# ziyaad30/ForwardTacotron

Measured on AMD Instinct MI355X. Metric: mel_frames_per_sec_train_step, higher is better.
Workload: dtype f32

## Files before the change

### forwardtacotron_amd/csrc/ft_lr.hip

```cpp
#include "ft_common.h"

namespace {

__global__ __launch_bounds__(64) void ft_lr_scan_kernel(float* dur, int Tx, int* cum, int* total) {
  const int b = blockIdx.x, lane = threadIdx.x;
  float* d = dur + (long)b * Tx;
  int* c = cum + (long)b * (Tx + 1);
  int carry = 0;
  for (int j0 = 0; j0 < Tx; j0 += 64) {
    int j = j0 + lane;
    int r = 0;
    if (j < Tx) {
      float v = d[j];
      if (v < 0.f) {
        v = 0.f;
        d[j] = 0.f;
      }
      r = (int)(long)(v + 0.5f);
    }
    int s = r;
#pragma unroll
    for (int o = 1; o < 64; o <<= 1) {
      int u = __shfl_up(s, o, 64);
      if (lane >= o) s += u;
    }
    if (j < Tx) c[j] = carry + s - r;
    carry += __shfl(s, 63, 64);
  }
  if (lane == 0) {
    c[Tx] = carry;
    total[b] = carry;
  }
}

__global__ __launch_bounds__(64) void ft_gen_durations_kernel(float* dur, const long* __restrict__ x_len, int Tx,
                                                              long* __restrict__ mel_len, int* bad) {
  const int b = blockIdx.x, lane = threadIdx.x;
  float* d = dur + (long)b * Tx;
  long Lb = x_len[b];
  if (Lb < 1 || Lb > Tx) {
    if (lane == 0) atomicOr(bad, 1);
    Lb = Lb < 1 ? 1 : Tx;
  }
  const int L = (int)Lb;
  long tr = 0;
  for (int j = lane; j < L; j += 64) tr += (long)d[j];
#pragma unroll
  for (int o = 32; o > 0; o >>= 1) tr += __shfl_xor(tr, o, 64);
  const bool fallback = tr <= 0;
  long total = 0;
  for (int j = lane; j < Tx; j += 64) {
    float v = 0.f;
    if (j < L) {
      v = fallback ? 2.f : d[j];
      if (v < 0.f) v = 0.f;
    }
    d[j] = v;
    total += (long)(v + 0.5f);
  }
#pragma unroll
  for (int o = 32; o > 0; o >>= 1) total += __shfl_xor(total, o, 64);
  if (lane == 0) mel_len[b] = total;
}

template <int FR>
__global__ __launch_bounds__(256) void ft_lr_expand_kernel(const float* __restrict__ x, const int* __restrict__ cum,
                                                           float* __restrict__ y, int* __restrict__ src_idx,
                                                           int Tx, int Tm, int C, int vec, long y_bs, long y_ts,
                                                           const float* __restrict__ pad_row) {
  __shared__ int src[FR];
  const int b = blockIdx.y;
  const int t0 = blockIdx.x * FR;
  const int* c = cum + (long)b * (Tx + 1);
  if (threadIdx.x < FR) {
    int t = t0 + threadIdx.x;
    int tok = -1;
    if (t < Tm && t < c[Tx]) {
      int lo = 0, hi = Tx - 1;
      while (lo < hi) {
        int mid = (lo + hi + 1) >> 1;
        if (c[mid] <= t) lo = mid; else hi = mid - 1;
      }
      tok = lo;
    }
    src[threadIdx.x] = tok;
    if (t < Tm && src_idx) src_idx[(long)b * Tm + t] = tok;
  }
  __syncthreads();
  const int wave = threadIdx.x >> 6, lane = threadIdx.x & 63;
  for (int f = wave; f < FR; f += 4) {
    int t = t0 + f;
    if (t >= Tm) break;
    int tok = src[f];
    float* yr = y + ((long)b * y_bs + (long)t * y_ts) * C;
    if (vec) {
      const float4* xr = reinterpret_cast<const float4*>(tok < 0 ? pad_row : x + ((long)b * Tx + tok) * C);
      float4* y4 = reinterpret_cast<float4*>(yr);
      for (int i = lane; i < C / 4; i += 64) y4[i] = xr ? xr[i] : make_float4(0.f, 0.f, 0.f, 0.f);
    } else {
      const float* xr = tok < 0 ? pad_row : x + ((long)b * Tx + tok) * C;
      for (int i = lane; i < C; i += 64) yr[i] = xr ? xr[i] : 0.f;
    }
  }
}

__global__ __launch_bounds__(256) void ft_lr_bwd_cols_kernel(const float* __restrict__ dy, const int* __restrict__ cum,
                                                             float* __restrict__ dx, float* __restrict__ dtail, int B,
                                                             int Tx, int Tm, int C, long dy_bs, long dy_ts) {
  const int wave = threadIdx.x >> 6, lane = threadIdx.x & 63;
  const long row = (long)blockIdx.x * 4 + wave;
  const int col = (blockIdx.y * 64 + lane) * 4;
  const long ntok = (long)B * Tx;
  if (row >= ntok + (dtail ? B : 0) || col >= C) return;
  const bool tail = row >= ntok;
  const int b = tail ? (int)(row - ntok) : (int)(row / Tx), j = tail ? Tx : (int)(row - (long)b * Tx);
  const int* c = cum + (long)b * (Tx + 1);
  int f0 = c[j], f1 = tail ? Tm : c[j + 1];
  if (f1 > Tm) f1 = Tm;
  float4 a = make_float4(0.f, 0.f, 0.f, 0.f);
  const float* src = dy + ((long)b * dy_bs + (long)f0 * dy_ts) * C + col;
  const long step = dy_ts * C;
  for (int t = f0; t < f1; t += 4, src += 4 * step) {
    const float4 z = make_float4(0.f, 0.f, 0.f, 0.f);
    const float4 g0 = *reinterpret_cast<const float4*>(src);
    const float4 g1 = t + 1 < f1 ? *reinterpret_cast<const float4*>(src + step) : z;
    const float4 g2 = t + 2 < f1 ? *reinterpret_cast<const float4*>(src + 2 * step) : z;
    const float4 g3 = t + 3 < f1 ? *reinterpret_cast<const float4*>(src + 3 * step) : z;
    a.x = (((a.x + g0.x) + g1.x) + g2.x) + g3.x;
    a.y = (((a.y + g0.y) + g1.y) + g2.y) + g3.y;
    a.z = (((a.z + g0.z) + g1.z) + g2.z) + g3.z;
    a.w = (((a.w + g0.w) + g1.w) + g2.w) + g3.w;
  }
  *reinterpret_cast<float4*>((tail ? dtail + (long)b * C : dx + row * C) + col) = a;
}

__global__ __launch_bounds__(256) void ft_lr_bwd_kernel(const float* __restrict__ dy, const int* __restrict__ cum,
                                                        float* __restrict__ dx, int B, int Tx, int Tm, int C, int vec) {
  const int wave = threadIdx.x >> 6, lane = threadIdx.x & 63;
  long row = (long)blockIdx.x * 4 + wave;
  if (row >= (long)B * Tx) return;
  int b = (int)(row / Tx), j = (int)(row - (long)b * Tx);
  const int* c = cum + (long)b * (Tx + 1);
  int f0 = c[j], f1 = c[j + 1];
  if (f1 > Tm) f1 = Tm;
  float* dxr = dx + row * C;
  if (vec) {
    for (int i = lane; i < C / 4; i += 64) {
      float4 a = make_float4(0.f, 0.f, 0.f, 0.f);
      for (int t = f0; t < f1; ++t) {
        float4 g = reinterpret_cast<const float4*>(dy + ((long)b * Tm + t) * C)[i];
        a.x += g.x; a.y += g.y; a.z += g.z; a.w += g.w;
      }
      reinterpret_cast<float4*>(dxr)[i] = a;
    }
  } else {
    for (int i = lane; i < C; i += 64) {
      float a = 0.f;
      for (int t = f0; t < f1; ++t) a += dy[((long)b * Tm + t) * C + i];
      dxr[i] = a;
    }
  }
}

}

int ft_gen_durations_impl(float* dur, const long* x_len, int B, int Tx, long* mel_len, int* bad, hipStream_t stream) {
  if (B <= 0) return FT_OK;
  hipLaunchKernelGGL(ft_gen_durations_kernel, dim3(B), dim3(64), 0, stream, dur, x_len, Tx, mel_len, bad);
  return ft_check_launch("gen_durations");
}

int ft_lr_scan_impl(float* dur, int B, int Tx, int* cum, int* total, hipStream_t stream) {
  FT_REQUIRE(B >= 0 && Tx >= 0, "lr_scan: bad dims");
  if (B == 0) return FT_OK;
  hipLaunchKernelGGL(ft_lr_scan_kernel, dim3(B), dim3(64), 0, stream, dur, Tx, cum, total);
  return ft_check_launch("lr_scan");
}

int ft_lr_expand_impl(const float* x, const int* cum, float* y, int* src_idx, int B, int Tx, int Tm, int C,
                      hipStream_t stream, int y_time_major, const float* pad_row) {
  FT_REQUIRE(B >= 0 && Tx >= 0 && Tm >= 0 && C >= 0, "lr_expand: bad dims");
  if (B == 0 || Tm == 0 || C == 0) return FT_OK;
  FT_REQUIRE(Tx > 0, "lr_expand: Tm > 0 requires Tx > 0");
  int vec = (C % 4 == 0) && ((uintptr_t)x % 16 == 0) && ((uintptr_t)y % 16 == 0) && ((uintptr_t)pad_row % 16 == 0);
  constexpr int FR = 16;
  hipLaunchKernelGGL(ft_lr_expand_kernel<FR>, dim3(ft_cdiv(Tm, FR), B), dim3(256), 0, stream, x, cum, y, src_idx,
                     Tx, Tm, C, vec, y_time_major ? 1L : (long)Tm, y_time_major ? (long)B : 1L, pad_row);
  return ft_check_launch("lr_expand");
}

int ft_lr_bwd_impl(const float* dy, const int* cum, float* dx, int B, int Tx, int Tm, int C, hipStream_t stream,
                   int dy_time_major, float* dtail) {
  FT_REQUIRE(B >= 0 && Tx >= 0 && Tm >= 0 && C >= 0, "lr_bwd: bad dims");
  if (B == 0 || Tx == 0 || C == 0) return FT_OK;
  int vec = (C % 4 == 0) && ((uintptr_t)dy % 16 == 0) && ((uintptr_t)dx % 16 == 0);
  if (dy_time_major || dtail || (vec && C >= 1024)) {
    FT_REQUIRE(vec && (uintptr_t)dtail % 16 == 0, "lr_bwd: this form needs C %% 4 == 0 and 16-byte aligned buffers");
    hipLaunchKernelGGL(ft_lr_bwd_cols_kernel, dim3(ft_cdiv((long)B * Tx + (dtail ? B : 0), 4), ft_cdiv(C, 256)), dim3(256),
                       0, stream, dy, cum, dx, dtail, B, Tx, Tm, C, dy_time_major ? 1L : (long)Tm,
                       dy_time_major ? (long)B : 1L);
    return ft_check_launch("lr_bwd");
  }
  hipLaunchKernelGGL(ft_lr_bwd_kernel, dim3(ft_cdiv((long)B * Tx, 4)), dim3(256), 0, stream, dy, cum, dx, B, Tx, Tm,
                     C, vec);
  return ft_check_launch("lr_bwd");
}
```

### forwardtacotron_amd/csrc/ft_rnn.hip

```cpp
#include <stdlib.h>

#include <string.h>

#include "ft_gemm.h"
#include "ft_rnn.h"

namespace {

__device__ __forceinline__ float4 ld4g(const float* p, int remaining, bool vec) {
  float4 v = make_float4(0.f, 0.f, 0.f, 0.f);
  if (remaining >= 4 && vec) {
    v = *reinterpret_cast<const float4*>(p);
  } else {
    if (remaining > 0) v.x = p[0];
    if (remaining > 1) v.y = p[1];
    if (remaining > 2) v.z = p[2];
    if (remaining > 3) v.w = p[3];
  }
  return v;
}

template <int MT, bool FAST>
__device__ __forceinline__ void wave_matmul(const float* const (&arow)[MT], const bool (&aok)[MT], const float* brow,
                                            bool bok, int K, int g0, int g1, int q, bool vec, f32x4 (&acc)[MT]) {
  for (int gb = g0; gb < g1; gb += GCH) {
    float4 av[MT][GCH], bv[GCH];
#pragma unroll
    for (int c = 0; c < GCH; ++c) {
      const int k = 16 * (gb + c) + 4 * q;
      if (FAST) {
        if (gb + c < g1) {
          bv[c] = *reinterpret_cast<const float4*>(brow + k);
#pragma unroll
          for (int m = 0; m < MT; ++m) av[m][c] = *reinterpret_cast<const float4*>(arow[m] + k);
        }
      } else {
        const bool in = (gb + c) < g1;
        bv[c] = ld4g(brow + k, (in && bok) ? K - k : 0, vec);
#pragma unroll
        for (int m = 0; m < MT; ++m) av[m][c] = ld4g(arow[m] + k, (in && aok[m]) ? K - k : 0, vec);
      }
    }
#pragma unroll
    for (int c = 0; c < GCH; ++c) {
      if (gb + c < g1) {
#pragma unroll
        for (int m = 0; m < MT; ++m) mfma4(av[m][c], bv[c], acc[m]);
      }
    }
  }
}

template <int G, int NW, int MT, bool FAST>
__global__ __launch_bounds__(NW * 64) void ft_rnn_fwd_step_kernel(RnnFwdArgs a) {
  constexpr int UB = 16 / G;
  __shared__ float red[NW * MT * 16 * RLD];
  const int d = blockIdx.z;
  const int u0 = blockIdx.x * UB;
  const int b0 = blockIdx.y * (MT * 16);
  const int tid = threadIdx.x, wave = tid >> 6, lane = tid & 63;
  const int q = lane >> 4, l15 = lane & 15;
  const int H = a.H, T = a.T, s = a.s;
  const long ldo = (long)a.ND * H;

  const int ci = tid / UB, cu = tid - ci * UB;
  const int cb = b0 + ci, cun = u0 + cu;
  bool cact = tid < MT * 16 * UB && cb < a.B && cun < H;
  int ct = 0;
  float xg[G], bg[G], prev = 0.f;
#pragma unroll
  for (int g = 0; g < G; ++g) xg[g] = bg[g] = 0.f;
  if (cact) {
    const int L = clamp_len(a.lens, cb, T);
    cact = s < L;
    if (cact) {
      ct = d == 0 ? s : L - 1 - s;
      const int tprev = d == 0 ? ct - 1 : ct + 1;
      const float* xr = a.xp + ((long)ct * a.B + cb) * ((long)a.ND * G * H) + (long)d * G * H + cun;
#pragma unroll
      for (int g = 0; g < G; ++g) {
        xg[g] = xr[(long)g * H];
        bg[g] = a.bhh[d][g * H + cun];
      }
      if (s > 0) {
        const long op = ((long)tprev * a.B + cb) * ldo + (long)d * H + cun;
        prev = G == 3 ? a.out[op] : a.cst[op];
      }
    }
  }

  f32x4 acc[MT];
#pragma unroll
  for (int m = 0; m < MT; ++m)
#pragma unroll
    for (int e = 0; e < 4; ++e) acc[m][e] = 0.f;

  if (s > 0) {
    const float* arow[MT];
    bool aok[MT];
#pragma unroll
    for (int m = 0; m < MT; ++m) {
      const int bA = b0 + m * 16 + l15;
      const int LA = bA < a.B ? clamp_len(a.lens, bA, T) : 0;
      aok[m] = bA < a.B && s < LA;
      const int tprev = d == 0 ? s - 1 : LA - s;
      const long row = aok[m] ? (long)tprev * a.B + bA : 0;
      arow[m] = a.out + row * ldo + (long)d * H;
    }
    const int gj = l15 / UB, ul = l15 - gj * UB;
    const bool bok = gj < G && (u0 + ul) < H;
    const float* brow = a.whh[d] + (bok ? ((long)gj * H + u0 + ul) * H : 0);
    const int ngroups = (H + 15) / 16;
    const int gpw = (ngroups + NW - 1) / NW;
    const int g0 = wave * gpw, g1 = min(ngroups, g0 + gpw);
    wave_matmul<MT, FAST>(arow, aok, brow, bok, H, g0, g1, q, a.vec, acc);
  }
  store_partials<MT>(red, wave, lane, acc);
  __syncthreads();

  if (cact) {
    float hp[G];
#pragma unroll
    for (int g = 0; g < G; ++g) {
      float v = 0.f;
#pragma unroll
      for (int w = 0; w < NW; ++w) v += red[w * (MT * 16 * RLD) + ci * RLD + g * UB + cu];
      hp[g] = v + bg[g];
    }
    const long o = ((long)ct * a.B + cb) * ldo + (long)d * H + cun;
    float* gs = a.gates ? a.gates + (((long)ct * a.B + cb) * a.ND + d) * 4 * H + cun : nullptr;
    if (G == 3) {
      float r = ft_sigmoid(xg[0] + hp[0]);
      float z = ft_sigmoid(xg[1] + hp[1]);
      float n = ft_tanh(xg[2] + r * hp[2]);
      a.out[o] = (1.f - z) * n + z * prev;
      if (gs) {
        gs[0] = r; gs[H] = z; gs[2 * H] = n; gs[3 * H] = hp[2];
      }
    } else {
      float ig = ft_sigmoid(xg[0] + hp[0]);
      float fg = ft_sigmoid(xg[1] + hp[1]);
      float gg = ft_tanh(xg[2] + hp[2]);
      float og = ft_sigmoid(xg[G - 1] + hp[G - 1]);
      float c = fg * prev + ig * gg;
      a.cst[o] = c;
      a.out[o] = og * ft_tanh(c);
      if (gs) {
        gs[0] = ig; gs[H] = fg; gs[2 * H] = gg; gs[3 * H] = og;
      }
    }
  }
}

template <int G, int NW, bool FAST>
__global__ __launch_bounds__(NW * 64) void ft_rnn_bwd_step_kernel(RnnBwdArgs a) {
  __shared__ float red[NW * 16 * RLD];
  const int d = blockIdx.z;
  const int u0 = blockIdx.x * 16;
  const int b0 = blockIdx.y * 16;
  const int tid = threadIdx.x, wave = tid >> 6, lane = tid & 63;
  const int q = lane >> 4, l15 = lane & 15;
  const int H = a.H, T = a.T, s = a.s, K = G * H;
  const long ldg = (long)a.ND * K;
  const long ldo = (long)a.ND * H;

  const int ci = tid >> 4, cj = tid & 15;
  const int cb = b0 + ci, cun = u0 + cj;
  bool cact = tid < 256 && cb < a.B && cun < H;
  int ct = 0;
  float gv[4] = {0.f, 0.f, 0.f, 0.f}, dov = 0.f, cin = 0.f, cc = 0.f, prev = 0.f;
  if (cact) {
    const int L = clamp_len(a.lens, cb, T);
    cact = s < L;
    if (cact) {
      ct = d == 0 ? L - 1 - s : s;
      const int tprev = d == 0 ? ct - 1 : ct + 1;
      const bool has_prev = tprev >= 0 && tprev < L;
      const long o = ((long)ct * a.B + cb) * ldo + (long)d * H + cun;
      const long op = ((long)tprev * a.B + cb) * ldo + (long)d * H + cun;
      const float* gs = a.gates + (((long)ct * a.B + cb) * a.ND + d) * 4 * H + cun;
#pragma unroll
      for (int g = 0; g < 4; ++g) gv[g] = gs[(long)g * H];
      dov = a.dout[o];
      if (s > 0) cin = a.carry[((long)cb * a.ND + d) * H + cun];
      if (G == 3) {
        prev = has_prev ? a.out[op] : 0.f;
      } else {
        cc = a.cst[o];
        prev = has_prev ? a.cst[op] : 0.f;
      }
    }
  }

  f32x4 acc[1];
#pragma unroll
  for (int e = 0; e < 4; ++e) acc[0][e] = 0.f;
  if (s > 0) {
    const int bA = b0 + l15;
    const int LA = bA < a.B ? clamp_len(a.lens, bA, T) : 0;
    const bool aok[1] = {bA < a.B && s < LA};
    const int tnext = d == 0 ? LA - s : s - 1;
    const long row = aok[0] ? (long)tnext * a.B + bA : 0;
    const float* arow[1] = {a.dhp + row * ldg + (long)d * K};
    const bool bok = (u0 + l15) < H;
    const float* brow = a.whhT[d] + (bok ? (long)(u0 + l15) * K : 0);
    const int ngroups = (K + 15) / 16;
    const int gpw = (ngroups + NW - 1) / NW;
    const int g0 = wave * gpw, g1 = min(ngroups, g0 + gpw);
    wave_matmul<1, FAST>(arow, aok, brow, bok, K, g0, g1, q, a.vec, acc);
  }
  store_partials<1>(red, wave, lane, acc);
  __syncthreads();

  if (cact) {
    float rec = 0.f;
#pragma unroll
    for (int w = 0; w < NW; ++w) rec += red[w * (16 * RLD) + ci * RLD + cj];
    float* cr = a.carry + ((long)cb * a.ND + d) * H + cun;
    float* dx = a.dxp + ((long)ct * a.B + cb) * ldg + (long)d * K + cun;
    if (G == 3) {
      const float dh = dov + rec + cin;
      const float r = gv[0], z = gv[1], n = gv[2], hn = gv[3];
      const float dz = dh * (prev - n) * z * (1.f - z);
      const float dn = dh * (1.f - z) * (1.f - n * n);
      const float dr = dn * hn * r * (1.f - r);
      dx[0] = dr; dx[H] = dz; dx[2 * H] = dn;
      float* dhh = a.dhp + ((long)ct * a.B + cb) * ldg + (long)d * K + cun;
      dhh[0] = dr; dhh[H] = dz; dhh[2 * H] = dn * r;
      *cr = dh * z;
    } else {
      const float dh = dov + rec;
      const float ig = gv[0], fg = gv[1], gg = gv[2], og = gv[3];
      const float tc = ft_tanh(cc);
      const float dc = dh * og * (1.f - tc * tc) + cin;
      dx[0] = dc * gg * ig * (1.f - ig);
      dx[H] = dc * prev * fg * (1.f - fg);
      dx[2 * H] = dc * ig * (1.f - gg * gg);
      dx[3 * H] = dh * tc * og * (1.f - og);
      *cr = dc * fg;
    }
  }
}

__global__ void ft_fill_padded_kernel(const float* __restrict__ raw, const long* __restrict__ lens,
                                      float* __restrict__ out, int B, int T, int C, float pad) {
  long i = (long)blockIdx.x * blockDim.x + threadIdx.x;
  long total = (long)B * T * C;
  if (i >= total) return;
  long row = i / C;
  int c = (int)(i - row * C);
  int b = (int)(row / T), t = (int)(row - (long)b * T);
  out[i] = (!lens || t < lens[b]) ? raw[((long)t * B + b) * C + c] : pad;
}
__global__ void ft_bt_transpose_kernel(const float* __restrict__ src, float* __restrict__ dst, int B, int T, int C,
                                       int dst_time_major) {
  long i = (long)blockIdx.x * blockDim.x + threadIdx.x;
  long total = (long)B * T * C;
  if (i >= total) return;
  long row = i / C;
  int c = (int)(i - row * C);
  if (dst_time_major) {
    int t = (int)(row / B), b = (int)(row - (long)t * B);
    dst[i] = src[((long)b * T + t) * C + c];
  } else {
    int b = (int)(row / T), t = (int)(row - (long)b * T);
    dst[i] = src[((long)t * B + b) * C + c];
  }
}
__global__ void ft_mask_rows_kernel(const float* __restrict__ src, const long* __restrict__ lens,
                                    float* __restrict__ dst, int B, int T, int C) {
  long i = (long)blockIdx.x * blockDim.x + threadIdx.x;
  long total = (long)B * T * C;
  if (i >= total) return;
  long row = i / C;
  int b = (int)(row / T), t = (int)(row - (long)b * T);
  dst[i] = t < lens[b] ? src[i] : 0.f;
}

template <int G, int NW, int MT>
void launch_fwd(bool fast, dim3 grid, hipStream_t stream, const RnnFwdArgs& a) {
  if (fast)
    hipLaunchKernelGGL((ft_rnn_fwd_step_kernel<G, NW, MT, true>), grid, dim3(NW * 64), 0, stream, a);
  else
    hipLaunchKernelGGL((ft_rnn_fwd_step_kernel<G, NW, MT, false>), grid, dim3(NW * 64), 0, stream, a);
}

template <int G, int ND = 2>
int rnn_fwd(const float* xp, const float* whh_f, const float* whh_r, const float* bhh_f, const float* bhh_r,
            float* out, float* cst, float* gates, const long* lens, int B, int T, int H, void* ws,
            size_t ws_bytes, hipStream_t stream, const unsigned* gate = nullptr, int gate_cs = 0,
            hipEvent_t xp_complete = nullptr) {
  RnnFwdArgs a;
  a.xp = xp; a.whh[0] = whh_f; a.whh[1] = whh_r; a.bhh[0] = bhh_f; a.bhh[1] = bhh_r;
  a.out = out; a.cst = cst; a.gates = gates; a.lens = lens;
  a.B = B; a.T = T; a.H = H; a.ND = ND; a.Bld = B;
  a.gate = gate; a.gate_cs = gate_cs;
  a.vec = (H % 4 == 0) && ((uintptr_t)out % 16 == 0) && ((uintptr_t)whh_f % 16 == 0) && ((uintptr_t)whh_r % 16 == 0);
  const bool fast = a.vec && (H % 16 == 0);
  {
    const int rc = ft_rnn_fwd_persistent(G, a, ws, ws_bytes, stream);
    if (rc != -1) return rc;
  }
  if (gate) {
    if (xp_complete) (void)hipStreamWaitEvent(stream, xp_complete, 0);
    a.gate = nullptr;
    a.gate_cs = 0;
  }
  constexpr int SLICE = 64;
  if (B > SLICE && a.vec && H % 16 == 0) {
    auto slice = [&](int bo) {
      RnnFwdArgs c = a;
      const long ldo = (long)a.ND * H;
      c.xp = a.xp + (long)bo * a.ND * G * H;
      c.out = a.out + bo * ldo;
      c.cst = a.cst ? a.cst + bo * ldo : nullptr;
      c.gates = a.gates ? a.gates + (long)bo * a.ND * 4 * H : nullptr;
      c.lens = a.lens ? a.lens + bo : nullptr;
      c.B = B - bo < SLICE ? B - bo : SLICE;
      return c;
    };
    int rc = ft_rnn_fwd_persistent(G, slice(0), ws, ws_bytes, stream);
    if (rc != -1) {
      for (int bo = SLICE; bo < B && rc == FT_OK; bo += SLICE) {
        rc = ft_rnn_fwd_persistent(G, slice(bo), ws, ws_bytes, stream);
        FT_REQUIRE(rc != -1, "rnn_fwd: a later batch slice was refused the persistent form the first one got");
      }
      return rc;
    }
  }
  if (lens) {
    (void)hipMemsetAsync(out, 0, sizeof(float) * (size_t)B * T * ND * H, stream);
    if (cst) (void)hipMemsetAsync(cst, 0, sizeof(float) * (size_t)B * T * ND * H, stream);
  }
  constexpr int UB = 16 / G;
  const bool two = B > 16;
  dim3 grid(ft_cdiv(H, UB), ft_cdiv(B, two ? 32 : 16), ND);
  const int ngroups = ft_cdiv(H, 16);
  for (int s = 0; s < T; ++s) {
    a.s = s;
    if (ngroups > 16) {
      if (two) launch_fwd<G, 8, 2>(fast, grid, stream, a);
      else launch_fwd<G, 8, 1>(fast, grid, stream, a);
    } else {
      if (two) launch_fwd<G, 4, 2>(fast, grid, stream, a);
      else launch_fwd<G, 4, 1>(fast, grid, stream, a);
    }
  }
  return ft_check_launch("rnn_fwd");
}

template <int G, int NW>
void launch_bwd(bool fast, dim3 grid, hipStream_t stream, const RnnBwdArgs& a) {
  if (fast)
    hipLaunchKernelGGL((ft_rnn_bwd_step_kernel<G, NW, true>), grid, dim3(NW * 64), 0, stream, a);
  else
    hipLaunchKernelGGL((ft_rnn_bwd_step_kernel<G, NW, false>), grid, dim3(NW * 64), 0, stream, a);
}

template <int G>
int rnn_bwd(const float* dout, const float* out, const float* cst, const float* gates, const float* whhT_f,
            const float* whhT_r, float* dxp, float* dhp, float* carry, const long* lens, int B, int T, int H,
            void* ws, size_t ws_bytes, hipStream_t stream) {
  RnnBwdArgs a;
  a.dout = dout; a.out = out; a.cst = cst; a.gates = gates; a.whhT[0] = whhT_f; a.whhT[1] = whhT_r;
  a.dxp = dxp; a.dhp = dhp; a.carry = carry; a.lens = lens;
  a.B = B; a.T = T; a.H = H; a.ND = 2;
  a.vec = (H % 4 == 0) && ((uintptr_t)dhp % 16 == 0) && ((uintptr_t)whhT_f % 16 == 0) &&
          ((uintptr_t)whhT_r % 16 == 0);
  const bool fast = a.vec && (((long)G * H) % 16 == 0);
  {
    const int rc = ft_rnn_bwd_persistent(G, a, ws, ws_bytes, stream);
    if (rc != -1) return rc;
  }
  if (lens) {
    (void)hipMemsetAsync(dxp, 0, sizeof(float) * (size_t)B * T * 2 * G * H, stream);
    if (dhp != dxp) (void)hipMemsetAsync(dhp, 0, sizeof(float) * (size_t)B * T * 2 * G * H, stream);
  }
  dim3 grid(ft_cdiv(H, 16), ft_cdiv(B, 16), 2);
  const int ngroups = ft_cdiv((long)G * H, 16);
  for (int s = 0; s < T; ++s) {
    a.s = s;
    if (ngroups > 64) launch_bwd<G, 16>(fast, grid, stream, a);
    else if (ngroups > 16) launch_bwd<G, 8>(fast, grid, stream, a);
    else launch_bwd<G, 4>(fast, grid, stream, a);
  }
  return ft_check_launch("rnn_bwd");
}

#define FT_HIP_OK(call)                                   \
  do {                                                    \
    if ((call) != hipSuccess) {                           \
      ft_set_error("rnn layer: %s failed", #call);        \
      return FT_ERR_HIP;                                  \
    }                                                     \
  } while (0)

__global__ void ft_gate_set_kernel(unsigned* word, unsigned value) {
  __hip_atomic_store(word, value, __ATOMIC_RELEASE, __HIP_MEMORY_SCOPE_AGENT);
}

hipEvent_t layer_event(int which) {
  int dev = 0;
  (void)hipGetDevice(&dev);
  static hipEvent_t ev[16][2] = {};
  if (dev < 0 || dev >= 16) return nullptr;
  hipEvent_t& e = ev[dev][which];
  if (!e && hipEventCreateWithFlags(&e, hipEventDisableTiming) != hipSuccess) e = nullptr;
  return e;
}

template <int G>
int rnn_layer_fwd(const float* x, int In, const float* const* wih, const float* const* bih, float* xp,
                  const float* whh_f, const float* whh_r, const float* bhh_f, const float* bhh_r, const long* lens,
                  float* out, float* cst, float* gates, int B, int T, int H, void* ws, size_t ws_bytes, unsigned* gate,
                  int nchunks, int rev_lead, hipStream_t stream, hipStream_t side) {
  const long ldy = 2L * G * H;
  auto project = [&](int d, int t0, int n, hipStream_t st) {
    FtGemmBatch b;
    memset(&b, 0, sizeof(b));
    FtGemmTask& t = b.t[0];
    t.A = x + (long)t0 * In; t.B = wih[d]; t.C = xp + (long)t0 * B * ldy + (long)d * G * H; t.bias = bih ? bih[d] : nullptr;
    t.lda = In; t.ldb = In; t.ldc = ldy;
    t.M = B * n; t.N = G * H; t.K = In; t.taps = 1;
    t.amap = FtRowMap{n, T, 1, n, 0, 0};
    t.cmap = FtRowMap{n, 1, B, n, 0, 0};
    b.force_tile = ft_rows_tile_is_big(2L * ft_cdiv((long)B * T, 128) * ft_cdiv(G * H, 128), B * T, G * H) ? 2 : 1;
    return ft_launch_gemm_rows(&b, 1, false, st);
  };
  int cs = nchunks > 1 ? (T + nchunks - 1) / nchunks : T;
  if (cs < 16) cs = 16;
  const int nc = T > 0 ? (T + cs - 1) / cs : 1;
  hipEvent_t ev0 = layer_event(0), ev1 = layer_event(1);
  const double fill = (nc >= 2 && side && gate) ? ft_rnn_fwd_xcd_fill(G, B, T, H, ws, ws_bytes) : -1.0;
  if (nc < 2 || !side || side == stream || !gate || !ev0 || !ev1 || fill < 0.0 || fill > 0.75) {
    int rc = project(0, 0, T, stream);
    if (rc == FT_OK) rc = project(1, 0, T, stream);
    if (rc != FT_OK) return rc;
    return rnn_fwd<G>(xp, whh_f, whh_r, bhh_f, bhh_r, out, cst, gates, lens, B, T, H, ws, ws_bytes, stream);
  }
  auto chunk = [&](int d, int j, hipStream_t st) {
    const int lo = d == 0 ? j * cs : (T - (j + 1) * cs > 0 ? T - (j + 1) * cs : 0);
    const int hi = d == 0 ? (lo + cs < T ? lo + cs : T) : T - j * cs;
    return project(d, lo, hi - lo, st);
  };
  (void)hipMemsetAsync(gate, 0, 2 * sizeof(unsigned), stream);
  int rc = chunk(0, 0, stream);
  if (rc == FT_OK) rc = chunk(1, 0, stream);
  if (rc != FT_OK) return rc;
  FT_HIP_OK(hipEventRecord(ev0, stream));
  FT_HIP_OK(hipStreamWaitEvent(side, ev0, 0));
  int next[2] = {1, 1};
  auto issue = [&](int d) {
    if (next[d] >= nc || rc != FT_OK) return;
    rc = chunk(d, next[d], side);
    hipLaunchKernelGGL(ft_gate_set_kernel, dim3(1), dim3(1), 0, side, gate + d, (unsigned)next[d]);
    ++next[d];
  };
  for (int i = 0; i < rev_lead; ++i) issue(1);
  while ((next[0] < nc || next[1] < nc) && rc == FT_OK) {
    issue(0);
    issue(1);
  }
  FT_HIP_OK(hipEventRecord(ev1, side));
  if (rc != FT_OK) {
    (void)hipStreamWaitEvent(stream, ev1, 0);
    return rc;
  }
  rc = rnn_fwd<G>(xp, whh_f, whh_r, bhh_f, bhh_r, out, cst, gates, lens, B, T, H, ws, ws_bytes, stream, gate, cs, ev1);
  (void)hipStreamWaitEvent(stream, ev1, 0);
  return rc;
}

}

extern "C" {

int ft_lstm_layer_fwd(const float* x, int in_f, const float* wih_f, const float* wih_r, const float* bih_f,
                      const float* bih_r, float* xp, const float* whh_f, const float* whh_r, const float* bhh_f,
                      const float* bhh_r, const long* lens, float* out_raw, float* cstate, float* gates, int B, int T,
                      int H, void* workspace, size_t workspace_bytes, unsigned* gate, int nchunks, int rev_lead,
                      void* stream, void* side_stream) {
  FT_REQUIRE(B > 0 && T >= 0 && H > 0 && in_f > 0, "lstm_layer_fwd: bad dims");
  const float* wih[2] = {wih_f, wih_r};
  const float* bih[2] = {bih_f, bih_r};
  return rnn_layer_fwd<4>(x, in_f, wih, bih, xp, whh_f, whh_r, bhh_f, bhh_r, lens, out_raw, cstate, gates, B, T, H,
                          workspace, workspace_bytes, gate, nchunks, rev_lead, (hipStream_t)stream,
                          (hipStream_t)side_stream);
}

int ft_gru_layer_fwd(const float* x, int in_f, const float* wih_f, const float* wih_r, const float* bih_f,
                     const float* bih_r, float* xp, const float* whh_f, const float* whh_r, const float* bhh_f,
                     const float* bhh_r, float* out, float* gates, int B, int T, int H, void* workspace,
                     size_t workspace_bytes, unsigned* gate, int nchunks, void* stream, void* side_stream) {
  FT_REQUIRE(B > 0 && T >= 0 && H > 0 && in_f > 0, "gru_layer_fwd: bad dims");
  const float* wih[2] = {wih_f, wih_r};
  const float* bih[2] = {bih_f, bih_r};
  return rnn_layer_fwd<3>(x, in_f, wih, bih, xp, whh_f, whh_r, bhh_f, bhh_r, nullptr, out, nullptr, gates, B, T, H,
                          workspace, workspace_bytes, gate, nchunks, 0, (hipStream_t)stream, (hipStream_t)side_stream);
}

int ft_gru_fwd(const float* xp, const float* whh_f, const float* whh_r, const float* bhh_f, const float* bhh_r,
               float* out, float* gates, int B, int T, int H, void* workspace, size_t workspace_bytes,
               void* stream) {
  FT_REQUIRE(B > 0 && T >= 0 && H > 0, "gru_fwd: bad dims");
  return rnn_fwd<3>(xp, whh_f, whh_r, bhh_f, bhh_r, out, nullptr, gates, nullptr, B, T, H, workspace,
                    workspace_bytes, (hipStream_t)stream);
}

int ft_gru_fwd_lens(const float* xp, const float* whh_f, const float* whh_r, const float* bhh_f, const float* bhh_r,
                    const long* lens, float* out, float* gates, int B, int T, int H, void* workspace,
                    size_t workspace_bytes, void* stream) {
  FT_REQUIRE(B > 0 && T >= 0 && H > 0 && lens != nullptr, "gru_fwd_lens: bad dims / null lens");
  return rnn_fwd<3>(xp, whh_f, whh_r, bhh_f, bhh_r, out, nullptr, gates, lens, B, T, H, workspace, workspace_bytes,
                    (hipStream_t)stream);
}

int ft_gru_layer_fwd_lens(const float* x, int in_f, const float* wih_f, const float* wih_r, const float* bih_f,
                          const float* bih_r, float* xp, const float* whh_f, const float* whh_r, const float* bhh_f,
                          const float* bhh_r, const long* lens, float* out, float* gates, int B, int T, int H,
                          void* workspace, size_t workspace_bytes, unsigned* gate, int nchunks, int rev_lead,
                          void* stream, void* side_stream) {
  FT_REQUIRE(B > 0 && T >= 0 && H > 0 && in_f > 0 && lens != nullptr, "gru_layer_fwd_lens: bad dims / null lens");
  const float* wih[2] = {wih_f, wih_r};
  const float* bih[2] = {bih_f, bih_r};
  return rnn_layer_fwd<3>(x, in_f, wih, bih, xp, whh_f, whh_r, bhh_f, bhh_r, lens, out, nullptr, gates, B, T, H,
                          workspace, workspace_bytes, gate, nchunks, rev_lead, (hipStream_t)stream,
                          (hipStream_t)side_stream);
}

int ft_gru_bwd(const float* dout, const float* out, const float* gates, const float* whhT_f, const float* whhT_r,
               float* dxp, float* dhp, float* carry, int B, int T, int H, void* workspace, size_t workspace_bytes,
               void* stream) {
  FT_REQUIRE(B > 0 && T >= 0 && H > 0, "gru_bwd: bad dims");
  return rnn_bwd<3>(dout, out, nullptr, gates, whhT_f, whhT_r, dxp, dhp, carry, nullptr, B, T, H, workspace,
                    workspace_bytes, (hipStream_t)stream);
}

int ft_lstm_fwd(const float* xp, const float* whh_f, const float* whh_r, const float* bhh_f, const float* bhh_r,
                const long* lens, float* out_raw, float* cstate, float* gates, int B, int T, int H,
                void* workspace, size_t workspace_bytes, void* stream) {
  FT_REQUIRE(B > 0 && T >= 0 && H > 0, "lstm_fwd: bad dims");
  hipStream_t s = (hipStream_t)stream;
  return rnn_fwd<4>(xp, whh_f, whh_r, bhh_f, bhh_r, out_raw, cstate, gates, lens, B, T, H, workspace,
                    workspace_bytes, s);
}

int ft_lstm_fwd_uni(const float* xp, const float* whh, const float* bhh, float* out_raw, float* cstate, int B, int T,
                    int H, void* workspace, size_t workspace_bytes, void* stream) {
  FT_REQUIRE(B > 0 && T >= 0 && H > 0, "lstm_fwd_uni: bad dims");
  return rnn_fwd<4, 1>(xp, whh, whh, bhh, bhh, out_raw, cstate, nullptr, nullptr, B, T, H, workspace, workspace_bytes,
                       (hipStream_t)stream);
}

int ft_lstm_bwd(const float* dout, const float* out_raw, const float* cstate, const float* gates,
                const float* whhT_f, const float* whhT_r, const long* lens, float* dgates, float* carry, int B, int T,
                int H, void* workspace, size_t workspace_bytes, void* stream) {
  FT_REQUIRE(B > 0 && T >= 0 && H > 0, "lstm_bwd: bad dims");
  hipStream_t s = (hipStream_t)stream;
  return rnn_bwd<4>(dout, out_raw, cstate, gates, whhT_f, whhT_r, dgates, dgates, carry, lens, B, T, H, workspace,
                    workspace_bytes, s);
}

int ft_fill_padded(const float* raw, const long* lens, float* out, int B, int T, int C, float pad, void* stream) {
  long total = (long)B * T * C;
  if (total <= 0) return FT_OK;
  hipLaunchKernelGGL(ft_fill_padded_kernel, dim3(ft_cdiv(total, 256)), dim3(256), 0, (hipStream_t)stream, raw, lens,
                     out, B, T, C, pad);
  return ft_check_launch("fill_padded");
}

int ft_bt_transpose(const float* src, float* dst, int B, int T, int C, int dst_time_major, void* stream) {
  long total = (long)B * T * C;
  if (total <= 0) return FT_OK;
  hipLaunchKernelGGL(ft_bt_transpose_kernel, dim3(ft_cdiv(total, 256)), dim3(256), 0, (hipStream_t)stream, src, dst, B,
                     T, C, dst_time_major);
  return ft_check_launch("bt_transpose");
}

int ft_mask_rows(const float* src, const long* lens, float* dst, int B, int T, int C, void* stream) {
  long total = (long)B * T * C;
  if (total <= 0) return FT_OK;
  hipLaunchKernelGGL(ft_mask_rows_kernel, dim3(ft_cdiv(total, 256)), dim3(256), 0, (hipStream_t)stream, src, lens, dst,
                     B, T, C);
  return ft_check_launch("mask_rows");
}

}
```

Before: 1.022 million.

## Raise memory-level parallelism in length-regulator and row layout kernels

The length-regulator expand copy is unrolled so each lane issues eight float4 loads before storing them. The backward column-sum kernel gets a new block mapping where each wave handles one token and a 256-column chunk, with separate tail blocks, and it loads 16 or 24 frames per batch. The elementwise fill_padded, bt_transpose and mask_rows kernels are replaced by one row-oriented, float4-vectorised kernel with unrolled loads. The aim is to keep more memory requests in flight and avoid per-element index division, at the cost of higher register use and more complex indexing. A lab benchmark script and a copy-yardstick kernel are added for measuring these passes.

Measured after the change: 1.033 million, median of 6. Within noise of the previous version (+1.0%).

```diff
diff --git a/forwardtacotron_amd/csrc/ft_lr.hip b/forwardtacotron_amd/csrc/ft_lr.hip
--- a/forwardtacotron_amd/csrc/ft_lr.hip
+++ b/forwardtacotron_amd/csrc/ft_lr.hip
@@ -62,6 +62,8 @@
   for (int o = 32; o > 0; o >>= 1) total += __shfl_xor(total, o, 64);
   if (lane == 0) mel_len[b] = total;
 }
+
+constexpr int LR_COPY = 8;
 
 template <int FR>
 __global__ __launch_bounds__(256) void ft_lr_expand_kernel(const float* __restrict__ x, const int* __restrict__ cum,
@@ -93,45 +95,89 @@
     if (t >= Tm) break;
     int tok = src[f];
     float* yr = y + ((long)b * y_bs + (long)t * y_ts) * C;
+    const float* xr = tok < 0 ? pad_row : x + ((long)b * Tx + tok) * C;
     if (vec) {
-      const float4* xr = reinterpret_cast<const float4*>(tok < 0 ? pad_row : x + ((long)b * Tx + tok) * C);
       float4* y4 = reinterpret_cast<float4*>(yr);
-      for (int i = lane; i < C / 4; i += 64) y4[i] = xr ? xr[i] : make_float4(0.f, 0.f, 0.f, 0.f);
+      const int n4 = C / 4;
+      if (xr) {
+        const float4* x4 = reinterpret_cast<const float4*>(xr);
+        int i = lane;
+        for (; i + (LR_COPY - 1) * 64 < n4; i += LR_COPY * 64) {
+          float4 v[LR_COPY];
+#pragma unroll
+          for (int k = 0; k < LR_COPY; ++k) v[k] = x4[i + k * 64];
+#pragma unroll
+          for (int k = 0; k < LR_COPY; ++k) y4[i + k * 64] = v[k];
+        }
+        for (; i < n4; i += 64) y4[i] = x4[i];
+      } else {
+        for (int i = lane; i < n4; i += 64) y4[i] = make_float4(0.f, 0.f, 0.f, 0.f);
+      }
     } else {
-      const float* xr = tok < 0 ? pad_row : x + ((long)b * Tx + tok) * C;
       for (int i = lane; i < C; i += 64) yr[i] = xr ? xr[i] : 0.f;
     }
   }
 }
+
+template <int D>
+__device__ __forceinline__ void lr_add_frames(float4& acc, const float* src, long step, int n) {
+  float4 g[D];
+  if (n == D) {
+#pragma unroll
+    for (int k = 0; k < D; ++k) g[k] = *reinterpret_cast<const float4*>(src + k * step);
+  } else {
+#pragma unroll
+    for (int k = 0; k < D; ++k)
+      g[k] = k < n ? *reinterpret_cast<const float4*>(src + k * step) : make_float4(0.f, 0.f, 0.f, 0.f);
+  }
+#pragma unroll
+  for (int k = 0; k < D; ++k)
+    if (k < n) {
+      acc.x += g[k].x; acc.y += g[k].y; acc.z += g[k].z; acc.w += g[k].w;
+    }
+}
+
+constexpr int LR_TOK_DEPTH = 16;
+constexpr int LR_TAIL_DEPTH = 24;
 
 __global__ __launch_bounds__(256) void ft_lr_bwd_cols_kernel(const float* __restrict__ dy, const int* __restrict__ cum,
                                                              float* __restrict__ dx, float* __restrict__ dtail, int B,
-                                                             int Tx, int Tm, int C, long dy_bs, long dy_ts) {
-  const int wave = threadIdx.x >> 6, lane = threadIdx.x & 63;
-  const long row = (long)blockIdx.x * 4 + wave;
-  const int col = (blockIdx.y * 64 + lane) * 4;
-  const long ntok = (long)B * Tx;
-  if (row >= ntok + (dtail ? B : 0) || col >= C) return;
-  const bool tail = row >= ntok;
-  const int b = tail ? (int)(row - ntok) : (int)(row / Tx), j = tail ? Tx : (int)(row - (long)b * Tx);
+                                                             int Tx, int Tm, int C, long dy_bs, long dy_ts, int ntail) {
+  const int wave = __builtin_amdgcn_readfirstlane(threadIdx.x >> 6), lane = threadIdx.x & 63;
+  const int nchunk = (C + 255) >> 8;
+  const bool tail = (int)blockIdx.x < ntail;
+  int b, j, chunk;
+  if (tail) {
+    const int w = blockIdx.x * 4 + wave;
+    b = w / nchunk;
+    chunk = w - b * nchunk;
+    j = Tx;
+    if (b >= B) return;
+  } else {
+    const int ncg = (nchunk + 3) >> 2;
+    const int id = blockIdx.x - ntail;
+    const int row = id / ncg;
+    chunk = (id - row * ncg) * 4 + wave;
+    b = row / Tx;
+    j = row - b * Tx;
+  }
+  const int col = (chunk * 64 + lane) * 4;
+  if (col >= C) return;
   const int* c = cum + (long)b * (Tx + 1);
-  int f0 = c[j], f1 = tail ? Tm : c[j + 1];
+  const int f0 = c[j];
+  int f1 = tail ? Tm : c[j + 1];
   if (f1 > Tm) f1 = Tm;
   float4 a = make_float4(0.f, 0.f, 0.f, 0.f);
   const float* src = dy + ((long)b * dy_bs + (long)f0 * dy_ts) * C + col;
   const long step = dy_ts * C;
-  for (int t = f0; t < f1; t += 4, src += 4 * step) {
-    const float4 z = make_float4(0.f, 0.f, 0.f, 0.f);
-    const float4 g0 = *reinterpret_cast<const float4*>(src);
-    const float4 g1 = t + 1 < f1 ? *reinterpret_cast<const float4*>(src + step) : z;
-    const float4 g2 = t + 2 < f1 ? *reinterpret_cast<const float4*>(src + 2 * step) : z;
-    const float4 g3 = t + 3 < f1 ? *reinterpret_cast<const float4*>(src + 3 * step) : z;
-    a.x = (((a.x + g0.x) + g1.x) + g2.x) + g3.x;
-    a.y = (((a.y + g0.y) + g1.y) + g2.y) + g3.y;
-    a.z = (((a.z + g0.z) + g1.z) + g2.z) + g3.z;
-    a.w = (((a.w + g0.w) + g1.w) + g2.w) + g3.w;
-  }
-  *reinterpret_cast<float4*>((tail ? dtail + (long)b * C : dx + row * C) + col) = a;
+  if (tail) {
+    for (int t = f0; t < f1; t += LR_TAIL_DEPTH, src += LR_TAIL_DEPTH * step)
+      lr_add_frames<LR_TAIL_DEPTH>(a, src, step, min(f1 - t, LR_TAIL_DEPTH));
+  } else {
+    for (int t = f0; t < f1; t += LR_TOK_DEPTH, src += LR_TOK_DEPTH * step)
+      lr_add_frames<LR_TOK_DEPTH>(a, src, step, min(f1 - t, LR_TOK_DEPTH));
+  }
+  *reinterpret_cast<float4*>((tail ? dtail + (long)b * C : dx + ((long)b * Tx + j) * C) + col) = a;
 }
 
 __global__ __launch_bounds__(256) void ft_lr_bwd_kernel(const float* __restrict__ dy, const int* __restrict__ cum,
@@ -196,9 +242,12 @@
   int vec = (C % 4 == 0) && ((uintptr_t)dy % 16 == 0) && ((uintptr_t)dx % 16 == 0);
   if (dy_time_major || dtail || (vec && C >= 1024)) {
     FT_REQUIRE(vec && (uintptr_t)dtail % 16 == 0, "lr_bwd: this form needs C %% 4 == 0 and 16-byte aligned buffers");
-    hipLaunchKernelGGL(ft_lr_bwd_cols_kernel, dim3(ft_cdiv((long)B * Tx + (dtail ? B : 0), 4), ft_cdiv(C, 256)), dim3(256),
-                       0, stream, dy, cum, dx, dtail, B, Tx, Tm, C, dy_time_major ? 1L : (long)Tm,
-                       dy_time_major ? (long)B : 1L);
+    const int nchunk = ft_cdiv(C, 256);
+    const long ntail = dtail ? ft_cdiv((long)B * nchunk, 4) : 0;
+    const long nblocks = ntail + (long)B * Tx * ft_cdiv(nchunk, 4);
+    FT_REQUIRE(nblocks <= 0x7fffffffL, "lr_bwd: too many rows for one launch");
+    hipLaunchKernelGGL(ft_lr_bwd_cols_kernel, dim3((unsigned)nblocks), dim3(256), 0, stream, dy, cum, dx, dtail, B, Tx, Tm,
+                       C, dy_time_major ? 1L : (long)Tm, dy_time_major ? (long)B : 1L, (int)ntail);
     return ft_check_launch("lr_bwd");
   }
   hipLaunchKernelGGL(ft_lr_bwd_kernel, dim3(ft_cdiv((long)B * Tx, 4)), dim3(256), 0, stream, dy, cum, dx, B, Tx, Tm,
diff --git a/forwardtacotron_amd/csrc/ft_rnn.hip b/forwardtacotron_amd/csrc/ft_rnn.hip
--- a/forwardtacotron_amd/csrc/ft_rnn.hip
+++ b/forwardtacotron_amd/csrc/ft_rnn.hip
@@ -242,39 +242,54 @@
   }
 }
 
-__global__ void ft_fill_padded_kernel(const float* __restrict__ raw, const long* __restrict__ lens,
-                                      float* __restrict__ out, int B, int T, int C, float pad) {
-  long i = (long)blockIdx.x * blockDim.x + threadIdx.x;
-  long total = (long)B * T * C;
-  if (i >= total) return;
-  long row = i / C;
-  int c = (int)(i - row * C);
-  int b = (int)(row / T), t = (int)(row - (long)b * T);
-  out[i] = (!lens || t < lens[b]) ? raw[((long)t * B + b) * C + c] : pad;
-}
-__global__ void ft_bt_transpose_kernel(const float* __restrict__ src, float* __restrict__ dst, int B, int T, int C,
-                                       int dst_time_major) {
-  long i = (long)blockIdx.x * blockDim.x + threadIdx.x;
-  long total = (long)B * T * C;
-  if (i >= total) return;
-  long row = i / C;
-  int c = (int)(i - row * C);
-  if (dst_time_major) {
-    int t = (int)(row / B), b = (int)(row - (long)t * B);
-    dst[i] = src[((long)b * T + t) * C + c];
-  } else {
-    int b = (int)(row / T), t = (int)(row - (long)b * T);
-    dst[i] = src[((long)t * B + b) * C + c];
-  }
-}
-__global__ void ft_mask_rows_kernel(const float* __restrict__ src, const long* __restrict__ lens,
-                                    float* __restrict__ dst, int B, int T, int C) {
-  long i = (long)blockIdx.x * blockDim.x + threadIdx.x;
-  long total = (long)B * T * C;
-  if (i >= total) return;
-  long row = i / C;
-  int b = (int)(row / T), t = (int)(row - (long)b * T);
-  dst[i] = t < lens[b] ? src[i] : 0.f;
+constexpr int RNN_ROWS_IF = 8;
+template <typename V>
+__global__ __launch_bounds__(256) void ft_rnn_rows_kernel(const V* __restrict__ src, const long* __restrict__ lens,
+                                                          V* __restrict__ dst, unsigned nrows, unsigned D, unsigned Sm,
+                                                          int n, int lg, V pad) {
+  const unsigned gw = blockIdx.x * 4u + (threadIdx.x >> 6);
+  const int lane = threadIdx.x & 63;
+  const unsigned r = (gw << (6 - lg)) + (lane >> lg);
+  if (r >= nrows) return;
+  const unsigned q = r / D, m = r - q * D;
+  V* d = dst + (long)r * n;
+  const int w = 1 << lg;
+  int i = lane & (w - 1);
+  if (lens && (long)m >= lens[q]) {
+    for (; i < n; i += w) d[i] = pad;
+    return;
+  }
+  const V* s = src + (Sm ? (long)m * Sm + q : (long)r) * n;
+  for (; i < n; i += RNN_ROWS_IF * w) {
+    V v[RNN_ROWS_IF];
+#pragma unroll
+    for (int k = 0; k < RNN_ROWS_IF; ++k) {
+      v[k] = pad;
+      if (i + k * w < n) v[k] = s[i + k * w];
+    }
+    asm volatile("" ::: "memory");
+#pragma unroll
+    for (int k = 0; k < RNN_ROWS_IF; ++k)
+      if (i + k * w < n) d[i + k * w] = v[k];
+  }
+}
+
+int rnn_rows_launch(const char* what, const float* src, const long* lens, float* dst, long nrows, int D, int Sm, int C,
+                    float pad, hipStream_t stream) {
+  FT_REQUIRE(nrows <= 0x7fffffffL, "%s: too many rows for one launch", what);
+  const bool vec = C % 4 == 0 && (uintptr_t)src % 16 == 0 && (uintptr_t)dst % 16 == 0;
+  const int n = vec ? C / 4 : C;
+  int lg = 0;
+  while (lg < 6 && (1 << lg) < n) ++lg;
+  const unsigned blocks = (unsigned)ft_cdiv(nrows, 4L << (6 - lg));
+  if (vec)
+    hipLaunchKernelGGL(ft_rnn_rows_kernel<float4>, dim3(blocks), dim3(256), 0, stream,
+                       reinterpret_cast<const float4*>(src), lens, reinterpret_cast<float4*>(dst), (unsigned)nrows,
+                       (unsigned)D, (unsigned)Sm, n, lg, make_float4(pad, pad, pad, pad));
+  else
+    hipLaunchKernelGGL(ft_rnn_rows_kernel<float>, dim3(blocks), dim3(256), 0, stream, src, lens, dst, (unsigned)nrows,
+                       (unsigned)D, (unsigned)Sm, n, lg, pad);
+  return ft_check_launch(what);
 }
 
 template <int G, int NW, int MT>
@@ -564,25 +579,20 @@
 int ft_fill_padded(const float* raw, const long* lens, float* out, int B, int T, int C, float pad, void* stream) {
   long total = (long)B * T * C;
   if (total <= 0) return FT_OK;
-  hipLaunchKernelGGL(ft_fill_padded_kernel, dim3(ft_cdiv(total, 256)), dim3(256), 0, (hipStream_t)stream, raw, lens,
-                     out, B, T, C, pad);
-  return ft_check_launch("fill_padded");
+  return rnn_rows_launch("fill_padded", raw, lens, out, (long)B * T, T, B, C, pad, (hipStream_t)stream);
 }
 
 int ft_bt_transpose(const float* src, float* dst, int B, int T, int C, int dst_time_major, void* stream) {
   long total = (long)B * T * C;
   if (total <= 0) return FT_OK;
-  hipLaunchKernelGGL(ft_bt_transpose_kernel, dim3(ft_cdiv(total, 256)), dim3(256), 0, (hipStream_t)stream, src, dst, B,
-                     T, C, dst_time_major);
-  return ft_check_launch("bt_transpose");
+  return rnn_rows_launch("bt_transpose", src, nullptr, dst, (long)B * T, dst_time_major ? B : T, dst_time_major ? T : B,
+                         C, 0.f, (hipStream_t)stream);
 }
 
 int ft_mask_rows(const float* src, const long* lens, float* dst, int B, int T, int C, void* stream) {
   long total = (long)B * T * C;
   if (total <= 0) return FT_OK;
-  hipLaunchKernelGGL(ft_mask_rows_kernel, dim3(ft_cdiv(total, 256)), dim3(256), 0, (hipStream_t)stream, src, lens, dst,
-                     B, T, C);
-  return ft_check_launch("mask_rows");
-}
-
-}
+  return rnn_rows_launch("mask_rows", src, lens, dst, (long)B * T, T, 0, C, 0.f, (hipStream_t)stream);
+}
+
+}
diff --git a/lab/layout_passes_us.py b/lab/layout_passes_us.py
--- /dev/null
+++ b/lab/layout_passes_us.py
@@ -0,0 +1,143 @@
+import argparse
+import ctypes
+import hashlib
+import json
+import os
+import statistics
+import sys
+
+import torch
+
+ROOT = os.path.dirname(os.path.dirname(os.path.abspath(__file__)))
+sys.path.insert(0, ROOT)
+
+from forwardtacotron_amd import _lib, data, hip
+
+
+def timed(fn, n, reps):
+    for _ in range(3):
+        fn()
+    out = []
+    for _ in range(reps):
+        e0, e1 = torch.cuda.Event(enable_timing=True), torch.cuda.Event(enable_timing=True)
+        e0.record()
+        for _ in range(n):
+            fn()
+        e1.record()
+        torch.cuda.synchronize()
+        out.append(e0.elapsed_time(e1) * 1e3 / n)
+    return statistics.median(out), min(out), max(out)
+
+
+def sha(*ts):
+    h = hashlib.sha1()
+    for t in ts:
+        h.update(t.detach().cpu().contiguous().numpy().tobytes())
+    return h.hexdigest()[:12]
+
+
+def main():
+    ap = argparse.ArgumentParser()
+    ap.add_argument('--reps', type=int, default=5)
+    ap.add_argument('--n', type=int, default=50)
+    ap.add_argument('--pack', action='store_true')
+    ap.add_argument('--bn', action='store_true')
+    ap.add_argument('--json', default=None)
+    args = ap.parse_args()
+    dev = torch.device('cuda')
+    so = os.path.join(ROOT, 'lab', 'libstream_copy.so')
+    if not os.path.exists(so):
+        raise SystemExit(f'{so} is missing: build it first (the command is in lab/stream_copy.hip)')
+    sc = ctypes.CDLL(so)
+    sc.stream_copy.argtypes = [ctypes.c_void_p, ctypes.c_void_p, ctypes.c_long, ctypes.c_void_p]
+    ybuf = torch.empty(2, 144 << 20, device=dev)
+
+    def yardstick(nbytes):
+        n16 = nbytes // 32
+        assert n16 * 16 <= ybuf[0].numel() * 4
+        a, b, s = ybuf[0].data_ptr(), ybuf[1].data_ptr(), hip._stream()
+        return timed(lambda: sc.stream_copy(a, b, n16, s), args.n, args.reps)
+
+    batch = data.synthetic_batch(B=32, Tmax=128, n_mels=80, seed=0)
+    B, Tx = batch['dur'].shape
+    Tm = int(batch['mel_len'].max())
+    mel_len = batch['mel_len'].to(dev)
+    n_frm, n_tok = int(batch['mel_len'].sum()), int((batch['dur'] > 0).sum())
+    cum, _ = hip.lr_scan(batch['dur'].clone().to(dev))
+    g = torch.Generator().manual_seed(1)
+    CW, CN = 4096, 1024
+    P = torch.randn(B, Tx, CW, generator=g).to(dev)
+    pad_row = torch.randn(CW, generator=g).to(dev)
+    dg = torch.randn(Tm, B, CW, generator=g).to(dev)
+    raw = torch.randn(Tm, B, CN, generator=g).to(dev)
+    dout = torch.randn(B, Tm, CN, generator=g).to(dev)
+    mel = torch.randn(B, Tm, 80, generator=g).to(dev)
+    rows = torch.empty(B * Tx + B, CW, device=dev)
+    st = hip._stream
+    rowb = lambda n, C: n * C * 4
+
+    def bwd_tm(tail):
+        _lib.call('ft_lr_bwd_tm', dg.data_ptr(), cum.data_ptr(), rows.data_ptr(),
+                  rows[B * Tx:].data_ptr() if tail else None, B, Tx, Tm, CW, st())
+
+    passes = [
+        ('lr_bwd_tm C4096 (with dtail)', lambda: bwd_tm(True), rowb(Tm * B + B * Tx + B, CW),
+         lambda: sha(hip.lr_bwd_tm(dg, cum, Tx)[1])),
+        ('lr_bwd_tm C4096 (no dtail)', lambda: bwd_tm(False), rowb(n_frm + B * Tx, CW),
+         lambda: sha(hip.lr_bwd_tm(dg, cum, Tx)[0])),
+        ('lr_expand_tm C4096 pad_row', lambda: hip.lr_expand_tm(P, cum, Tm, pad_row), rowb(Tm * B + n_tok + 1, CW),
+         lambda: sha(hip.lr_expand_tm(P, cum, Tm, pad_row))),
+        ('lr_expand C4096 (batch-major)', lambda: hip.lr_expand(P, cum, Tm), rowb(Tm * B + n_tok, CW),
+         lambda: sha(*hip.lr_expand(P, cum, Tm, want_src=True))),
+        ('fill_padded C1024 lens', lambda: hip.fill_padded(raw, mel_len, -11.5), rowb(Tm * B + n_frm, CN),
+         lambda: sha(hip.fill_padded(raw, mel_len, -11.5))),
+        ('bt_transpose C1024 -> time-major', lambda: hip.bt_transpose(dout, True), rowb(2 * Tm * B, CN),
+         lambda: sha(hip.bt_transpose(dout, True), hip.bt_transpose(raw, False))),
+        ('mask_rows C80 (mel)', lambda: hip.mask_rows(mel, mel_len), rowb(Tm * B + n_frm, 80),
+         lambda: sha(hip.mask_rows(mel, mel_len))),
+    ]
+    if args.pack:
+        from forwardtacotron_amd.model import ForwardTacotron
+        from forwardtacotron_amd.trainer import TrainStep
+        torch.manual_seed(0)
+        ts = TrainStep(ForwardTacotron(**dict(data.SINGLESPEAKER_MODEL)).to(dev), lr=5e-5,
+                       train_cfg=dict(data.SINGLESPEAKER_TRAIN))
+        pk = ts._weight_packs()
+        outs = (list(pk.t2d.values()) + list(pk.wp.values()) + list(pk.wpt.values()) + list(pk.hw.values())
+                + [t for pair in pk.bank.values() for t in pair])
+        srcs = (list(pk.t2d.values()) + list(pk.wp.values()) + list(pk.hw.values())
+                + [pair[0] for pair in pk.bank.values()])
+        passes.append(('pack_weights (benchmark model)', pk.refresh,
+                       4 * (sum(t.numel() for t in outs) + sum(t.numel() for t in srcs)), lambda: sha(*outs)))
+
+    if args.bn:
+        Cb, grp = 2048, 256
+        y = torch.randn(B, Tm + 1, Cb, generator=g).to(dev)
+        do = torch.randn(B, Tm, Cb, generator=g).to(dev)
+        ga, be = torch.rand(Cb, generator=g).to(dev) + 0.5, torch.randn(Cb, generator=g).to(dev)
+        _, mean, rstd = hip.bn_train_fwd(y, ga, be, torch.zeros(Cb, device=dev), torch.ones(Cb, device=dev), Tm, grp)
+        nb = rowb(2 * B * Tm + 3 * B * (Tm + 1), Cb)
+        passes.append(('bn_bwd bank (partial4 + apply4)', lambda: hip.bn_bwd(do, y, ga, mean, rstd, grp, True), nb,
+                       lambda: sha(*hip.bn_bwd(do, y, ga, mean, rstd, grp, True))))
+        passes.append(('bn_pool_bwd bank (same + pool)', lambda: hip.bn_pool_bwd(do, y, ga, be, mean, rstd, grp, True), nb,
+                       lambda: sha(*hip.bn_pool_bwd(do, y, ga, be, mean, rstd, grp, True))))
+
+    res = []
+    print(f'library: {_lib.LIB_PATH}')
+    print(f'B {B} Tx {Tx} Tm {Tm} frames {n_frm} tokens with frames {n_tok}; {args.n} launches per event pair, '
+          f'{args.reps} pairs: median (min .. max)')
+    for name, fn, nbytes, digest in passes:
+        us, lo, hi = timed(fn, args.n, args.reps)
+        yus, ylo, yhi = yardstick(nbytes)
+        d = digest()
+        print(f'{name:34s} | {us:7.1f} us ({lo:7.1f} .. {hi:7.1f}) | {nbytes / 1e6:7.1f} MB | {nbytes / us / 1e3:6.0f} GB/s | '
+              f'copy {yus:6.1f} us ({ylo:6.1f} .. {yhi:6.1f}) {nbytes / yus / 1e3:6.0f} GB/s | share {yus / us:4.2f} | sha {d}',
+              flush=True)
+        res.append({'pass': name, 'us': us, 'min': lo, 'max': hi, 'bytes': nbytes, 'copy_us': yus, 'sha': d})
+    if args.json:
+        with open(args.json, 'w') as f:
+            json.dump({'library': _lib.LIB_PATH, 'passes': res}, f, indent=1)
+
+
+if __name__ == '__main__':
+    main()
diff --git a/lab/stream_copy.hip b/lab/stream_copy.hip
--- /dev/null
+++ b/lab/stream_copy.hip
@@ -0,0 +1,25 @@
+#include <hip/hip_runtime.h>
+
+namespace {
+constexpr int UNROLL = 4;
+__global__ __launch_bounds__(256) void stream_copy_kernel(const float4* __restrict__ src, float4* __restrict__ dst,
+                                                          long n16) {
+  long i = (long)blockIdx.x * (256 * UNROLL) + threadIdx.x;
+  float4 v[UNROLL];
+#pragma unroll
+  for (int k = 0; k < UNROLL; ++k)
+    if (i + k * 256 < n16) v[k] = src[i + k * 256];
+#pragma unroll
+  for (int k = 0; k < UNROLL; ++k)
+    if (i + k * 256 < n16) dst[i + k * 256] = v[k];
+}
+}
+
+extern "C" int stream_copy(const void* src, void* dst, long n16, void* stream) {
+  if (n16 <= 0) return 0;
+  const long blocks = (n16 + 256 * UNROLL - 1) / (256 * UNROLL);
+  if (blocks > 0x7fffffffL) return 1;
+  hipLaunchKernelGGL(stream_copy_kernel, dim3((unsigned)blocks), dim3(256), 0, (hipStream_t)stream,
+                     static_cast<const float4*>(src), static_cast<float4*>(dst), n16);
+  return hipGetLastError() == hipSuccess ? 0 : 2;
+}
```
